# marqo-ai/marqo

Hardware: NVIDIA H100
Metric: embeddings/s (open_clip/ViT-L-14 image vectorise, batch 256 per GPU) (higher is better)
Workload: dtype bf16

## Files before the change

marqo_b200/csrc/gemm.cu:

```cuda
#include "gemm.cuh"

#include <mutex>

#include "ptx.cuh"

namespace mb {
namespace gemm {

constexpr int BM = 128;
constexpr int BN = 128;
constexpr int BK = 64;
constexpr int WG_K = 16;
constexpr int STAGES = 3;
constexpr int MMA_THREADS = 256;
constexpr uint32_t A_STAGE_BYTES = BM * BK * 2;
constexpr uint32_t B_STAGE_BYTES = BN * BK * 2;
constexpr uint32_t STAGE_BYTES = A_STAGE_BYTES + B_STAGE_BYTES;
constexpr uint32_t BARRIER_BYTES = 256;
constexpr size_t SMEM_BYTES = (size_t)STAGES * STAGE_BYTES + 1024  + BARRIER_BYTES + 2 * BN * 4 ;
constexpr int EPI_ROWS = BM / 2;
constexpr uint32_t EPI_BOX_BYTES = EPI_ROWS * 128;
static_assert(4 * EPI_BOX_BYTES == STAGE_BYTES, "a warpgroup's fp32 64 x 128 block is one ring stage");

template <bool GATHER>
constexpr int threads() { return MMA_THREADS + (GATHER ? 128 : 32); }

struct Params {
    int M, N, K;
    int tiles_n;
    Epilogue ep;
    const uint8_t* img;
    int g;
    int patch;
    int row_bytes;
    int seg;
    int kbpd;
    float nscale[3], nshift[3];
};

__device__ __forceinline__ float ex2_approx(float x) {
    float y;
    asm("ex2.approx.ftz.f32 %0, %1;" : "=f"(y) : "f"(x));
    return y;
}

__device__ __forceinline__ float gelu_erf(float x) {
    const float a = x * 0.70710678118654752440f;
    const float t = fabsf(a);
    const float s = a * a;
    float r = fmaf(-2.49374837e-5f, t, 5.52836593e-4f);
    const float u = fmaf(-5.60337594e-3f, t, 3.49920232e-2f);
    r = fmaf(r, s, u);
    r = fmaf(r, t, -1.54047912e-1f);
    r = fmaf(r, t, -9.15890168e-1f);
    r = fmaf(r, t, -1.85700115e-1f);
    r = fmaf(r, t, -1.44269504f * t);
    const float e = copysignf(1.0f - ex2_approx(r), a);
    const float hx = 0.5f * x;
    return fmaf(hx, e, hx);
}

__device__ __forceinline__ __half2 gelu_erf_h2(__half2 x) {
    const __half2 a = __hmul2(x, __float2half2_rn(0.70710678118654752440f));
    const __half2 t = __habs2(a);
    const __half2 s = __hmul2(a, a);
    __half2 r = __hfma2(__float2half2_rn(-2.49374837e-5f), t, __float2half2_rn(5.52836593e-4f));
    const __half2 u = __hfma2(__float2half2_rn(-5.60337594e-3f), t, __float2half2_rn(3.49920232e-2f));
    r = __hfma2(r, s, u);
    r = __hfma2(r, t, __float2half2_rn(-1.54047912e-1f));
    r = __hfma2(r, t, __float2half2_rn(-9.15890168e-1f));
    r = __hfma2(r, t, __float2half2_rn(-1.85700115e-1f));
    r = __hfma2(r, t, __hmul2(t, __float2half2_rn(-1.44269504f)));
    const __half2 e = h2exp2(r);
    const __half2 om = __hsub2(__float2half2_rn(1.0f), e);
    const uint32_t eb = (*reinterpret_cast<const uint32_t*>(&om) & 0x7fff7fffu) | (*reinterpret_cast<const uint32_t*>(&a) & 0x80008000u);
    const __half2 erfv = *reinterpret_cast<const __half2*>(&eb);
    const __half2 hx = __hmul2(x, __float2half2_rn(0.5f));
    return __hfma2(hx, erfv, hx);
}

__device__ __forceinline__ float quick_gelu(float x) {
    return x / (1.0f + ex2_approx(-1.702f * 1.44269504f * x));
}

__device__ __forceinline__ uint32_t pack_bf16x2(float lo, float hi) {
    __nv_bfloat162 v = __floats2bfloat162_rn(lo, hi);
    return *reinterpret_cast<uint32_t*>(&v);
}

__device__ __forceinline__ uint32_t sw128_offset(int row, int unit) {
    return (uint32_t)row * 128u + (uint32_t)((unit ^ (row & 7)) << 4);
}

template <int ELEM>
__device__ __forceinline__ uint32_t epi_offset(int row, int col) {
    constexpr int BOX_COLS = 128 / ELEM;
    const int byte = (col % BOX_COLS) * ELEM;
    return (uint32_t)(col / BOX_COLS) * EPI_BOX_BYTES + sw128_offset(row, byte >> 4) + (uint32_t)(byte & 15);
}

__device__ __forceinline__ void warpgroup_sync(int wg) {
    if (wg == 0)
        ptx::bar_sync<1, 128>();
    else
        ptx::bar_sync<2, 128>();
}

template <bool GATHER, bool STAGED>
__global__ void __launch_bounds__(threads<GATHER>(), GATHER ? 1 : 2)
gemm_kernel(const __grid_constant__ CUtensorMap tmap_a, const __grid_constant__ CUtensorMap tmap_b,
            const __grid_constant__ CUtensorMap tmap_r, const __grid_constant__ CUtensorMap tmap_o, Params p) {
    static_assert(!(GATHER && STAGED), "the patch embed scatters token rows: register epilogue");
    extern __shared__ uint8_t smem_raw[];
    uint8_t* smem = reinterpret_cast<uint8_t*>((reinterpret_cast<uintptr_t>(smem_raw) + 1023) & ~uintptr_t(1023));
    uint64_t* full = reinterpret_cast<uint64_t*>(smem + (size_t)STAGES * STAGE_BYTES);
    uint64_t* empty = full + STAGES;
    float* bias_s = reinterpret_cast<float*>(smem + (size_t)STAGES * STAGE_BYTES + BARRIER_BYTES);

    const int warp = __shfl_sync(0xffffffffu, threadIdx.x >> 5, 0);
    const int lane = threadIdx.x & 31;
    const int tile_m = blockIdx.x / p.tiles_n, tile_n = blockIdx.x % p.tiles_n;
    const int m0 = tile_m * BM, n0 = tile_n * BN;
    const int kblocks = p.K / BK;

    if (threadIdx.x == MMA_THREADS) {
        ptx::prefetch_tmap(&tmap_b);
        if (!GATHER) ptx::prefetch_tmap(&tmap_a);
        if (STAGED) {
            ptx::prefetch_tmap(&tmap_o);
            if (p.ep.residual) ptx::prefetch_tmap(&tmap_r);
        }
        for (int i = 0; i < STAGES; ++i) {
            ptx::mbar_init(&full[i], GATHER ? 1 + 128 : 1);
            ptx::mbar_init(&empty[i], MMA_THREADS / 32);
        }
        ptx::fence_barrier_init();
    }
    __syncthreads();

    if (threadIdx.x >= MMA_THREADS) {
        const int pt = threadIdx.x - MMA_THREADS;
        if (!GATHER && pt >= 32) return;
        const uint8_t* prow = nullptr;
        if (GATHER) {
            const int r = m0 + pt;
            if (r < p.M) {
                const int gg = p.g * p.g;
                const int b = r / gg, pi = r - b * gg;
                const int py = pi / p.g, px = pi - py * p.g;
                prow = p.img + ((size_t)b * p.g * p.patch + (size_t)py * p.patch) * p.row_bytes + (size_t)px * p.patch * 3;
            }
        }
        for (int kb = 0; kb < kblocks; ++kb) {
            const int stage = kb % STAGES;
            const uint32_t phase = (uint32_t)(kb / STAGES) & 1u;
            uint8_t* sa = smem + (size_t)stage * STAGE_BYTES;
            uint8_t* sb = sa + A_STAGE_BYTES;
            ptx::mbar_wait(&empty[stage], phase ^ 1);
            if (pt == 0) {
                ptx::mbar_arrive_expect_tx(&full[stage], GATHER ? B_STAGE_BYTES : STAGE_BYTES);
                if (!GATHER) ptx::tma_load_2d(sa, &tmap_a, &full[stage], kb * BK, m0, ptx::kEvictNormal);
                ptx::tma_load_2d(sb, &tmap_b, &full[stage], kb * BK, n0, ptx::kEvictLast);
            }
            if (GATHER) {
                const int dy = kb / p.kbpd, j0 = (kb - dy * p.kbpd) * 64;
                const uint8_t* src = prow ? prow + (size_t)dy * p.row_bytes + j0 : nullptr;
                int c = j0 % 3;
#pragma unroll 1
                for (int u = 0; u < 8; ++u) {
                    uint32_t w[4];
#pragma unroll
                    for (int e = 0; e < 4; ++e) {
                        float v[2];
#pragma unroll
                        for (int h = 0; h < 2; ++h) {
                            const int j = u * 8 + e * 2 + h;
                            v[h] = (src != nullptr && j0 + j < p.seg) ? fmaf((float)__ldg(src + j), p.nscale[c], p.nshift[c]) : 0.f;
                            c = c == 2 ? 0 : c + 1;
                        }
                        w[e] = pack_bf16x2(v[0], v[1]);
                    }
                    *reinterpret_cast<uint4*>(sa + sw128_offset(pt, u)) = make_uint4(w[0], w[1], w[2], w[3]);
                }
                ptx::fence_proxy_async_smem();
                ptx::mbar_arrive(&full[stage]);
            }
        }
        if (STAGED) {
            for (int wg = 0; wg < 2; ++wg) {
                const int kb = kblocks + wg;
                const int stage = kb % STAGES;
                uint8_t* s = smem + (size_t)stage * STAGE_BYTES;
                ptx::mbar_wait(&empty[stage], ((uint32_t)(kb / STAGES) & 1u) ^ 1);
                if (pt != 0) continue;
                const int row0 = m0 + EPI_ROWS * wg;
                const int boxes = p.ep.residual != nullptr && row0 < p.M ? min(4, (p.N - n0) / 32) : 0;
                ptx::mbar_arrive_expect_tx(&full[stage], (uint32_t)boxes * EPI_BOX_BYTES);
                for (int b = 0; b < boxes; ++b)
                    ptx::tma_load_2d(s + b * EPI_BOX_BYTES, &tmap_r, &full[stage], n0 + 32 * b, row0, ptx::kEvictNormal);
            }
        }
        return;
    }

    const int wg = warp >> 2;
    const Epilogue& ep = p.ep;
    float bias_t = 0.f;
    if (STAGED && ep.bias != nullptr && n0 + (int)(threadIdx.x & 127) < p.N) bias_t = __ldg(ep.bias + n0 + (threadIdx.x & 127));
    float acc[BN / 2];
#pragma unroll
    for (int i = 0; i < BN / 2; ++i) acc[i] = 0.f;
    for (int kb = 0; kb < kblocks; ++kb) {
        const int stage = kb % STAGES;
        ptx::mbar_wait(&full[stage], (uint32_t)(kb / STAGES) & 1u);
        const uint32_t a_base = ptx::smem_u32(smem + (size_t)stage * STAGE_BYTES) + wg * (64 * 128);
        const uint32_t b_base = ptx::smem_u32(smem + (size_t)stage * STAGE_BYTES + A_STAGE_BYTES);
        ptx::wgmma_fence();
#pragma unroll
        for (int k = 0; k < BK / WG_K; ++k)
            ptx::wgmma_m64n128k16_bf16(acc, ptx::make_desc_k_sw128(a_base + k * WG_K * 2),
                                       ptx::make_desc_k_sw128(b_base + k * WG_K * 2), (kb | k) != 0 ? 1u : 0u);
        ptx::wgmma_commit();
        ptx::wgmma_wait<1>();
        if (kb > 0 && lane == 0) ptx::mbar_arrive(&empty[(kb - 1) % STAGES]);
    }
    ptx::wgmma_wait<0>();

    if constexpr (STAGED) {
        const int t = threadIdx.x & 127;
        float* wbias = bias_s + wg * BN;
        wbias[t] = bias_t;
        const int kb = kblocks + wg;
        ptx::mbar_wait(&full[kb % STAGES], (uint32_t)(kb / STAGES) & 1u);
        uint8_t* tile = smem + (size_t)(kb % STAGES) * STAGE_BYTES;
        warpgroup_sync(wg);
        const int rbase = (warp & 3) * 16 + (lane >> 2);
        const bool half_gelu = ep.act == ACT_GELU && !ep.act_fp32 && !ep.out_fp32;
#pragma unroll
        for (int i = 0; i < BN / 8; ++i) {
            const int col = 8 * i + 2 * (lane & 3);
            const float2 bv = *reinterpret_cast<const float2*>(wbias + col);
#pragma unroll
            for (int h = 0; h < 2; ++h) {
                const int r = rbase + 8 * h;
                float x0 = acc[4 * i + 2 * h] + bv.x, x1 = acc[4 * i + 2 * h + 1] + bv.y;
                if (half_gelu) {
                    const float2 y = __half22float2(gelu_erf_h2(__floats2half2_rn(x0, x1)));
                    *reinterpret_cast<uint32_t*>(tile + epi_offset<2>(r, col)) = pack_bf16x2(y.x, y.y);
                    continue;
                }
                if (ep.act == ACT_GELU) {
                    x0 = gelu_erf(x0);
                    x1 = gelu_erf(x1);
                } else if (ep.act == ACT_QUICKGELU) {
                    x0 = quick_gelu(x0);
                    x1 = quick_gelu(x1);
                }
                if (ep.out_fp32) {
                    float2* dst = reinterpret_cast<float2*>(tile + epi_offset<4>(r, col));
                    if (ep.residual) {
                        const float2 rv = *dst;
                        x0 += rv.x;
                        x1 += rv.y;
                    }
                    *dst = make_float2(x0, x1);
                } else {
                    *reinterpret_cast<uint32_t*>(tile + epi_offset<2>(r, col)) = pack_bf16x2(x0, x1);
                }
            }
        }
        ptx::fence_proxy_async_smem();
        warpgroup_sync(wg);
        const int row0 = m0 + EPI_ROWS * wg;
        if (t == 0 && row0 < p.M) {
            const int box_cols = ep.out_fp32 ? 32 : 64;
            for (int b = 0; b * box_cols < BN && n0 + b * box_cols < p.N; ++b)
                ptx::tma_store_2d(&tmap_o, tile + b * EPI_BOX_BYTES, n0 + b * box_cols, row0);
            ptx::tma_store_commit();
            ptx::tma_store_wait_read<0>();
        }
    } else {
        const int rbase = m0 + wg * 64 + (warp & 3) * 16 + (lane >> 2);
        long long orow[2];
        bool rok[2];
#pragma unroll
        for (int h = 0; h < 2; ++h) {
            const int r = rbase + 8 * h;
            const int b = r / ep.remap_group;
            rok[h] = r < p.M;
            orow[h] = (long long)b * (ep.remap_group + 1) + 1 + (r - b * ep.remap_group);
        }
#pragma unroll
        for (int i = 0; i < BN / 8; ++i) {
            const int col = n0 + 8 * i + 2 * (lane & 3);
            if (col >= p.N) continue;
            float2 bv = make_float2(0.f, 0.f);
            if (ep.bias) bv = __ldg(reinterpret_cast<const float2*>(ep.bias + col));
#pragma unroll
            for (int h = 0; h < 2; ++h) {
                if (!rok[h]) continue;
                const int r = rbase + 8 * h;
                float x0 = acc[4 * i + 2 * h] + bv.x, x1 = acc[4 * i + 2 * h + 1] + bv.y;
                if (ep.act == ACT_GELU) {
                    x0 = gelu_erf(x0);
                    x1 = gelu_erf(x1);
                } else if (ep.act == ACT_QUICKGELU) {
                    x0 = quick_gelu(x0);
                    x1 = quick_gelu(x1);
                }
                if (ep.rowbias) {
                    const float2 pb =
                        __ldg(reinterpret_cast<const float2*>(ep.rowbias + (size_t)(1 + r % ep.remap_group) * p.N + col));
                    x0 += pb.x;
                    x1 += pb.y;
                }
                *reinterpret_cast<float2*>(static_cast<float*>(ep.out) + orow[h] * ep.ldo + col) = make_float2(x0, x1);
            }
        }
    }
}

void configure() {
    static std::once_flag once;
    std::call_once(once, [] {
        const auto attr = cudaFuncAttributeMaxDynamicSharedMemorySize;
        MB_CUDA(cudaFuncSetAttribute(gemm_kernel<false, true>, attr, (int)SMEM_BYTES));
        MB_CUDA(cudaFuncSetAttribute(gemm_kernel<false, false>, attr, (int)SMEM_BYTES));
        MB_CUDA(cudaFuncSetAttribute(gemm_kernel<true, false>, attr, (int)SMEM_BYTES));
    });
}

template <bool GATHER, bool STAGED>
static void launch_tiles(const __nv_bfloat16* A, int lda, const __nv_bfloat16* W, int M, int N, int K, const Epilogue& ep,
                         cudaStream_t stream, const PatchGather* pg = nullptr) {
    Params p{};
    if (GATHER) {
        p.img = pg->img;
        p.patch = pg->patch;
        p.g = pg->S / pg->patch;
        p.row_bytes = 3 * pg->S;
        p.seg = 3 * pg->patch;
        p.kbpd = patch_gather_kbpd(pg->patch);
        for (int c = 0; c < 3; ++c) {
            p.nscale[c] = (float)(1.0 / (255.0 * (double)pg->std[c]));
            p.nshift[c] = (float)(-(double)pg->mean[c] / (double)pg->std[c]);
        }
    }
    p.M = M;
    p.N = N;
    p.K = K;
    p.tiles_n = (N + BN - 1) / BN;
    p.ep = ep;
    const long long tiles = (long long)((M + BM - 1) / BM) * p.tiles_n;
    if (tiles > 0x7fffffffLL) fail(B200_ERR_UNSUPPORTED, "gemm: %lld tiles is too many", tiles);
    CUtensorMap tb = make_tmap_2d(W, CU_TENSOR_MAP_DATA_TYPE_BFLOAT16, 2, (uint64_t)K, (uint64_t)N, (uint64_t)K * 2, BK, BN,
                                  CU_TENSOR_MAP_SWIZZLE_128B);
    CUtensorMap ta = GATHER ? tb
                            : make_tmap_2d(A, CU_TENSOR_MAP_DATA_TYPE_BFLOAT16, 2, (uint64_t)K, (uint64_t)M,
                                           (uint64_t)lda * 2, BK, BM, CU_TENSOR_MAP_SWIZZLE_128B);
    CUtensorMap tr = tb, to = tb;
    if (STAGED) {
        if (ep.residual)
            tr = make_tmap_2d(ep.residual, CU_TENSOR_MAP_DATA_TYPE_FLOAT32, 4, (uint64_t)N, (uint64_t)M,
                              (uint64_t)ep.ldr * 4, 32, EPI_ROWS, CU_TENSOR_MAP_SWIZZLE_128B);
        to = ep.out_fp32 ? make_tmap_2d(ep.out, CU_TENSOR_MAP_DATA_TYPE_FLOAT32, 4, (uint64_t)N, (uint64_t)M,
                                        (uint64_t)ep.ldo * 4, 32, EPI_ROWS, CU_TENSOR_MAP_SWIZZLE_128B)
                         : make_tmap_2d(ep.out, CU_TENSOR_MAP_DATA_TYPE_BFLOAT16, 2, (uint64_t)N, (uint64_t)M,
                                        (uint64_t)ep.ldo * 2, 64, EPI_ROWS, CU_TENSOR_MAP_SWIZZLE_128B);
    }
    gemm_kernel<GATHER, STAGED><<<(unsigned)tiles, threads<GATHER>(), SMEM_BYTES, stream>>>(ta, tb, tr, to, p);
    MB_CUDA(cudaGetLastError());
}

bool patch_gather_supported(int S, int patch) {
    return S > 0 && patch > 0 && S % patch == 0;
}

void launch_patch_embed(const PatchGather& pg, const __nv_bfloat16* Wg, int N, const Epilogue& ep, int sms,
                        cudaStream_t stream) {
    (void)sms;
    if (pg.n <= 0 || N <= 0) return;
    if (!patch_gather_supported(pg.S, pg.patch))
        fail(B200_ERR_INTERNAL, "patch gather: image %d / patch %d is not supported", pg.S, pg.patch);
    if (N % 32 != 0 || ep.ldo % 8 != 0) fail(B200_ERR_INTERNAL, "patch gather: N = %d, ldo = %d", N, ep.ldo);
    if (ep.remap_group <= 0 || ep.residual != nullptr || !ep.out_fp32)
        fail(B200_ERR_INTERNAL, "patch gather: token scatter to fp32 output without residual only");
    configure();
    const int g = pg.S / pg.patch;
    const long long M = (long long)pg.n * g * g;
    if (M > 0x7fffffffLL) fail(B200_ERR_INVALID_ARG, "patch gather: batch of %d images is too large", pg.n);
    launch_tiles<true, false>(nullptr, 0, Wg, (int)M, N, patch_gather_k(pg.patch), ep, stream, &pg);
}

void launch(const __nv_bfloat16* A, int lda, const __nv_bfloat16* W, int M, int N, int K, const Epilogue& ep, int sms,
            cudaStream_t stream) {
    (void)sms;
    if (M <= 0 || N <= 0) return;
    if (K <= 0 || K % BK != 0) fail(B200_ERR_INTERNAL, "gemm: K = %d must be a positive multiple of %d", K, BK);
    if (N % 32 != 0) fail(B200_ERR_INTERNAL, "gemm: N = %d must be a multiple of 32", N);
    if (lda % 8 != 0 || ep.ldo % 8 != 0) fail(B200_ERR_INTERNAL, "gemm: leading dimensions must be multiples of 8");
    if (ep.remap_group > 0) {
        if (ep.residual != nullptr || !ep.out_fp32)
            fail(B200_ERR_INTERNAL, "gemm: token scatter to fp32 output without residual only");
        configure();
        launch_tiles<false, false>(A, lda, W, M, N, K, ep, stream);
        return;
    }
    if ((reinterpret_cast<uintptr_t>(ep.out) & 15) != 0) fail(B200_ERR_INTERNAL, "gemm: output not 16-byte aligned");
    if (ep.rowbias != nullptr) fail(B200_ERR_INTERNAL, "gemm: the positional bias goes with the token scatter");
    if (ep.residual != nullptr &&
        (!ep.out_fp32 || ep.ldr % 4 != 0 || (reinterpret_cast<uintptr_t>(ep.residual) & 15) != 0))
        fail(B200_ERR_INTERNAL, "gemm: the residual needs an fp32 output, ldr %% 4 == 0 and 16-byte alignment");
    configure();
    launch_tiles<false, true>(A, lda, W, M, N, K, ep, stream);
}

}
}
```

marqo_b200/csrc/ptx.cuh:

```cuda
#pragma once
#include <cstdint>
#include <cstdio>
#include <cuda.h>
#include <cuda_runtime.h>

namespace ptx {

__device__ __forceinline__ uint32_t smem_u32(const void* p) {
    return static_cast<uint32_t>(__cvta_generic_to_shared(p));
}

__device__ __forceinline__ uint32_t lane_id() {
    uint32_t l;
    asm volatile("mov.u32 %0, %%laneid;" : "=r"(l));
    return l;
}

__device__ __forceinline__ uint64_t globaltimer_ns() {
    uint64_t t;
    asm volatile("mov.u64 %0, %%globaltimer;" : "=l"(t));
    return t;
}

__device__ __forceinline__ bool elect_one() {
    uint32_t pred;
    asm volatile(
        "{\n"
        ".reg .pred p;\n"
        "elect.sync _|p, 0xffffffff;\n"
        "selp.u32 %0, 1, 0, p;\n"
        "}\n"
        : "=r"(pred));
    return pred != 0;
}

__device__ __forceinline__ void mbar_init(uint64_t* bar, uint32_t count) {
    asm volatile("mbarrier.init.shared::cta.b64 [%0], %1;" ::"r"(smem_u32(bar)), "r"(count) : "memory");
}
__device__ __forceinline__ void fence_barrier_init() {
    asm volatile("fence.mbarrier_init.release.cluster;" ::: "memory");
}
__device__ __forceinline__ void fence_proxy_async_smem() {
    asm volatile("fence.proxy.async.shared::cta;" ::: "memory");
}
__device__ __forceinline__ void mbar_arrive_expect_tx(uint64_t* bar, uint32_t bytes) {
    asm volatile("mbarrier.arrive.expect_tx.shared::cta.b64 _, [%0], %1;" ::"r"(smem_u32(bar)), "r"(bytes)
                 : "memory");
}
__device__ __forceinline__ void mbar_arrive(uint64_t* bar) {
    asm volatile("mbarrier.arrive.shared::cta.b64 _, [%0];" ::"r"(smem_u32(bar)) : "memory");
}
__device__ __forceinline__ bool mbar_try_wait(uint64_t* bar, uint32_t parity) {
    uint32_t ok;
    asm volatile(
        "{\n"
        ".reg .pred p;\n"
        "mbarrier.try_wait.parity.shared::cta.b64 p, [%1], %2;\n"
        "selp.u32 %0, 1, 0, p;\n"
        "}\n"
        : "=r"(ok)
        : "r"(smem_u32(bar)), "r"(parity)
        : "memory");
    return ok != 0;
}
__device__ __forceinline__ void mbar_wait(uint64_t* bar, uint32_t parity) {
    if (mbar_try_wait(bar, parity)) return;
    uint64_t t0 = globaltimer_ns();
    uint32_t spins = 0;
    while (!mbar_try_wait(bar, parity)) {
        if ((++spins & 0x3ff) == 0 && globaltimer_ns() - t0 > 4000000000ull) __trap();
    }
}

constexpr uint64_t kEvictNormal = 0x1000000000000000ull;
constexpr uint64_t kEvictFirst = 0x12F0000000000000ull;
constexpr uint64_t kEvictLast = 0x14F0000000000000ull;

__device__ __forceinline__ void prefetch_tmap(const CUtensorMap* tmap) {
    asm volatile("prefetch.tensormap [%0];" ::"l"(reinterpret_cast<uint64_t>(tmap)) : "memory");
}

__device__ __forceinline__ void tma_load_2d(void* smem_dst, const CUtensorMap* tmap, uint64_t* bar, int32_t c0,
                                            int32_t c1, uint64_t cache_hint) {
    asm volatile(
        "cp.async.bulk.tensor.2d.shared::cluster.global.tile.mbarrier::complete_tx::bytes.L2::cache_hint"
        " [%0], [%1, {%3, %4}], [%2], %5;"
        ::"r"(smem_u32(smem_dst)), "l"(reinterpret_cast<uint64_t>(tmap)), "r"(smem_u32(bar)), "r"(c0), "r"(c1),
        "l"(cache_hint)
        : "memory");
}

__device__ __forceinline__ void tma_store_2d(const CUtensorMap* tmap, const void* smem_src, int32_t c0, int32_t c1) {
    asm volatile("cp.async.bulk.tensor.2d.global.shared::cta.tile.bulk_group [%0, {%2, %3}], [%1];" ::"l"(
                     reinterpret_cast<uint64_t>(tmap)),
                 "r"(smem_u32(smem_src)), "r"(c0), "r"(c1)
                 : "memory");
}
__device__ __forceinline__ void tma_store_commit() { asm volatile("cp.async.bulk.commit_group;" ::: "memory"); }
template <int N>
__device__ __forceinline__ void tma_store_wait_read() {
    asm volatile("cp.async.bulk.wait_group.read %0;" ::"n"(N) : "memory");
}
template <int N>
__device__ __forceinline__ void tma_store_wait() {
    asm volatile("cp.async.bulk.wait_group %0;" ::"n"(N) : "memory");
}

__device__ __forceinline__ uint64_t make_desc_k_sw128(uint32_t smem_addr) {
    uint64_t d = 0;
    d |= static_cast<uint64_t>((smem_addr & 0x3FFFF) >> 4);
    d |= static_cast<uint64_t>(1) << 16;
    d |= static_cast<uint64_t>(1024 >> 4) << 32;
    d |= static_cast<uint64_t>(1) << 62;
    return d;
}

__device__ __forceinline__ uint64_t make_desc_mn_sw128(uint32_t smem_addr, uint32_t lbo_bytes) {
    uint64_t d = 0;
    d |= static_cast<uint64_t>((smem_addr & 0x3FFFF) >> 4);
    d |= static_cast<uint64_t>((lbo_bytes >> 4) & 0x3FFF) << 16;
    d |= static_cast<uint64_t>(1024 >> 4) << 32;
    d |= static_cast<uint64_t>(1) << 62;
    return d;
}

__device__ __forceinline__ uint64_t make_desc_k_sw64(uint32_t smem_addr) {
    uint64_t d = 0;
    d |= static_cast<uint64_t>((smem_addr & 0x3FFFF) >> 4);
    d |= static_cast<uint64_t>(1) << 16;
    d |= static_cast<uint64_t>(512 >> 4) << 32;
    d |= static_cast<uint64_t>(2) << 62;
    return d;
}

__device__ __forceinline__ uint64_t make_desc_mn_sw64(uint32_t smem_addr, uint32_t lbo_bytes) {
    uint64_t d = 0;
    d |= static_cast<uint64_t>((smem_addr & 0x3FFFF) >> 4);
    d |= static_cast<uint64_t>((lbo_bytes >> 4) & 0x3FFF) << 16;
    d |= static_cast<uint64_t>(512 >> 4) << 32;
    d |= static_cast<uint64_t>(2) << 62;
    return d;
}

__device__ __forceinline__ void wgmma_fence() { asm volatile("wgmma.fence.sync.aligned;" ::: "memory"); }
__device__ __forceinline__ void wgmma_commit() { asm volatile("wgmma.commit_group.sync.aligned;" ::: "memory"); }
template <int N>
__device__ __forceinline__ void wgmma_wait() {
    asm volatile("wgmma.wait_group.sync.aligned %0;" ::"n"(N) : "memory");
}

__device__ __forceinline__ void wgmma_m64n128k16_f16(float (&d)[64], uint64_t desc_a, uint64_t desc_b, uint32_t scale_d) {
    asm volatile(
        "{\n"
        ".reg .pred p;\n"
        "setp.ne.b32 p, %66, 0;\n"
        "wgmma.mma_async.sync.aligned.m64n128k16.f32.f16.f16 "
        "{"
        "%0, %1, %2, %3, %4, %5, %6, %7, %8, %9, %10, %11, %12, %13, %14, %15, "
        "%16, %17, %18, %19, %20, %21, %22, %23, %24, %25, %26, %27, %28, %29, %30, %31, "
        "%32, %33, %34, %35, %36, %37, %38, %39, %40, %41, %42, %43, %44, %45, %46, %47, "
        "%48, %49, %50, %51, %52, %53, %54, %55, %56, %57, %58, %59, %60, %61, %62, %63"
        "}, %64, %65, p, 1, 1, 0, 0;\n"
        "}\n"
        : "+f"(d[0]), "+f"(d[1]), "+f"(d[2]), "+f"(d[3]), "+f"(d[4]), "+f"(d[5]), "+f"(d[6]), "+f"(d[7]),
          "+f"(d[8]), "+f"(d[9]), "+f"(d[10]), "+f"(d[11]), "+f"(d[12]), "+f"(d[13]), "+f"(d[14]), "+f"(d[15]),
          "+f"(d[16]), "+f"(d[17]), "+f"(d[18]), "+f"(d[19]), "+f"(d[20]), "+f"(d[21]), "+f"(d[22]), "+f"(d[23]),
          "+f"(d[24]), "+f"(d[25]), "+f"(d[26]), "+f"(d[27]), "+f"(d[28]), "+f"(d[29]), "+f"(d[30]), "+f"(d[31]),
          "+f"(d[32]), "+f"(d[33]), "+f"(d[34]), "+f"(d[35]), "+f"(d[36]), "+f"(d[37]), "+f"(d[38]), "+f"(d[39]),
          "+f"(d[40]), "+f"(d[41]), "+f"(d[42]), "+f"(d[43]), "+f"(d[44]), "+f"(d[45]), "+f"(d[46]), "+f"(d[47]),
          "+f"(d[48]), "+f"(d[49]), "+f"(d[50]), "+f"(d[51]), "+f"(d[52]), "+f"(d[53]), "+f"(d[54]), "+f"(d[55]),
          "+f"(d[56]), "+f"(d[57]), "+f"(d[58]), "+f"(d[59]), "+f"(d[60]), "+f"(d[61]), "+f"(d[62]), "+f"(d[63])
        : "l"(desc_a), "l"(desc_b), "r"(scale_d));
}
__device__ __forceinline__ void wgmma_m64n128k16_bf16(float (&d)[64], uint64_t desc_a, uint64_t desc_b, uint32_t scale_d) {
    asm volatile(
        "{\n"
        ".reg .pred p;\n"
        "setp.ne.b32 p, %66, 0;\n"
        "wgmma.mma_async.sync.aligned.m64n128k16.f32.bf16.bf16 "
        "{"
        "%0, %1, %2, %3, %4, %5, %6, %7, %8, %9, %10, %11, %12, %13, %14, %15, "
        "%16, %17, %18, %19, %20, %21, %22, %23, %24, %25, %26, %27, %28, %29, %30, %31, "
        "%32, %33, %34, %35, %36, %37, %38, %39, %40, %41, %42, %43, %44, %45, %46, %47, "
        "%48, %49, %50, %51, %52, %53, %54, %55, %56, %57, %58, %59, %60, %61, %62, %63"
        "}, %64, %65, p, 1, 1, 0, 0;\n"
        "}\n"
        : "+f"(d[0]), "+f"(d[1]), "+f"(d[2]), "+f"(d[3]), "+f"(d[4]), "+f"(d[5]), "+f"(d[6]), "+f"(d[7]),
          "+f"(d[8]), "+f"(d[9]), "+f"(d[10]), "+f"(d[11]), "+f"(d[12]), "+f"(d[13]), "+f"(d[14]), "+f"(d[15]),
          "+f"(d[16]), "+f"(d[17]), "+f"(d[18]), "+f"(d[19]), "+f"(d[20]), "+f"(d[21]), "+f"(d[22]), "+f"(d[23]),
          "+f"(d[24]), "+f"(d[25]), "+f"(d[26]), "+f"(d[27]), "+f"(d[28]), "+f"(d[29]), "+f"(d[30]), "+f"(d[31]),
          "+f"(d[32]), "+f"(d[33]), "+f"(d[34]), "+f"(d[35]), "+f"(d[36]), "+f"(d[37]), "+f"(d[38]), "+f"(d[39]),
          "+f"(d[40]), "+f"(d[41]), "+f"(d[42]), "+f"(d[43]), "+f"(d[44]), "+f"(d[45]), "+f"(d[46]), "+f"(d[47]),
          "+f"(d[48]), "+f"(d[49]), "+f"(d[50]), "+f"(d[51]), "+f"(d[52]), "+f"(d[53]), "+f"(d[54]), "+f"(d[55]),
          "+f"(d[56]), "+f"(d[57]), "+f"(d[58]), "+f"(d[59]), "+f"(d[60]), "+f"(d[61]), "+f"(d[62]), "+f"(d[63])
        : "l"(desc_a), "l"(desc_b), "r"(scale_d));
}
__device__ __forceinline__ void wgmma_m64n64k16_bf16_rs_tb(float (&d)[32], const uint32_t (&a)[4], uint64_t desc_b, uint32_t scale_d) {
    asm volatile(
        "{\n"
        ".reg .pred p;\n"
        "setp.ne.b32 p, %37, 0;\n"
        "wgmma.mma_async.sync.aligned.m64n64k16.f32.bf16.bf16 "
        "{"
        "%0, %1, %2, %3, %4, %5, %6, %7, %8, %9, %10, %11, %12, %13, %14, %15, "
        "%16, %17, %18, %19, %20, %21, %22, %23, %24, %25, %26, %27, %28, %29, %30, %31"
        "}, {%32, %33, %34, %35}, %36, p, 1, 1, 1;\n"
        "}\n"
        : "+f"(d[0]), "+f"(d[1]), "+f"(d[2]), "+f"(d[3]), "+f"(d[4]), "+f"(d[5]), "+f"(d[6]), "+f"(d[7]),
          "+f"(d[8]), "+f"(d[9]), "+f"(d[10]), "+f"(d[11]), "+f"(d[12]), "+f"(d[13]), "+f"(d[14]), "+f"(d[15]),
          "+f"(d[16]), "+f"(d[17]), "+f"(d[18]), "+f"(d[19]), "+f"(d[20]), "+f"(d[21]), "+f"(d[22]), "+f"(d[23]),
          "+f"(d[24]), "+f"(d[25]), "+f"(d[26]), "+f"(d[27]), "+f"(d[28]), "+f"(d[29]), "+f"(d[30]), "+f"(d[31])
        : "r"(a[0]), "r"(a[1]), "r"(a[2]), "r"(a[3]), "l"(desc_b), "r"(scale_d));
}
__device__ __forceinline__ void wgmma_m64n32k16_bf16_rs_tb(float (&d)[16], const uint32_t (&a)[4], uint64_t desc_b, uint32_t scale_d) {
    asm volatile(
        "{\n"
        ".reg .pred p;\n"
        "setp.ne.b32 p, %21, 0;\n"
        "wgmma.mma_async.sync.aligned.m64n32k16.f32.bf16.bf16 "
        "{"
        "%0, %1, %2, %3, %4, %5, %6, %7, %8, %9, %10, %11, %12, %13, %14, %15"
        "}, {%16, %17, %18, %19}, %20, p, 1, 1, 1;\n"
        "}\n"
        : "+f"(d[0]), "+f"(d[1]), "+f"(d[2]), "+f"(d[3]), "+f"(d[4]), "+f"(d[5]), "+f"(d[6]), "+f"(d[7]),
          "+f"(d[8]), "+f"(d[9]), "+f"(d[10]), "+f"(d[11]), "+f"(d[12]), "+f"(d[13]), "+f"(d[14]), "+f"(d[15])
        : "r"(a[0]), "r"(a[1]), "r"(a[2]), "r"(a[3]), "l"(desc_b), "r"(scale_d));
}
template <int ID, int COUNT>
__device__ __forceinline__ void bar_sync() {
    asm volatile("bar.sync %0, %1;" ::"n"(ID), "n"(COUNT) : "memory");
}

}
```

Baseline: 1877.

## Add persistent warp-specialized 128x256 GEMM kernel for large-K projections

Adds a persistent GEMM kernel with a 128x256 tile using m64n256k16 wgmma, a single-thread TMA producer warpgroup with reduced registers via setmaxnreg, and two consumer warpgroups with double epilogue buffers. It also adds residual TMA loads, L2 prefetch of the residual and a packed fp16 GELU path for bf16 outputs. It is dispatched when K >= 1024, N is a multiple of 256 and there are at least as many tiles as SMs. The aim is higher operand reuse per tile and less launch and tail overhead for the big ViT-L MLP and attention projections. The cost is heavy register pressure (128 fp32 accumulators per thread) and a serialized epilogue that is not overlapped with the next tile's MMA.

```diff
diff --git a/marqo_b200/csrc/gemm.cu b/marqo_b200/csrc/gemm.cu
--- a/marqo_b200/csrc/gemm.cu
+++ b/marqo_b200/csrc/gemm.cu
@@ -22,12 +22,23 @@
 constexpr uint32_t EPI_BOX_BYTES = EPI_ROWS * 128;
 static_assert(4 * EPI_BOX_BYTES == STAGE_BYTES, "a warpgroup's fp32 64 x 128 block is one ring stage");
 
+constexpr int P_BN = 256;
+constexpr int P_STAGES = 3;
+constexpr uint32_t P_STAGE_BYTES = A_STAGE_BYTES + P_BN * BK * 2;
+constexpr uint32_t P_RING_BYTES = P_STAGES * P_STAGE_BYTES;
+constexpr uint32_t EPI_BYTES = 4 * EPI_BOX_BYTES;
+constexpr int PERSISTENT_THREADS = 128 + MMA_THREADS;
+constexpr int ACT_GELU_H2 = 3;
+constexpr size_t P_SMEM_BYTES = 1024  + P_RING_BYTES + 2 * EPI_BYTES + 2 * P_BN * 4 + BARRIER_BYTES;
+static_assert(P_SMEM_BYTES <= 227 * 1024, "over the opt-in shared memory of an H100 CTA");
+static_assert(P_BN * 2 * EPI_ROWS == EPI_BYTES, "a warpgroup's bf16 64 x 256 block is one epilogue buffer");
+
 template <bool GATHER>
 constexpr int threads() { return MMA_THREADS + (GATHER ? 128 : 32); }
 
 struct Params {
     int M, N, K;
-    int tiles_n;
+    int tiles_m, tiles_n;
     Epilogue ep;
     const uint8_t* img;
     int g;
@@ -320,6 +331,201 @@
     }
 }
 
+template <bool OUT_FP32, int ACT>
+__global__ void __launch_bounds__(PERSISTENT_THREADS, 1)
+gemm_persistent_kernel(const __grid_constant__ CUtensorMap tmap_a, const __grid_constant__ CUtensorMap tmap_b,
+                       const __grid_constant__ CUtensorMap tmap_r, const __grid_constant__ CUtensorMap tmap_o, Params p) {
+    extern __shared__ uint8_t smem_raw[];
+    uint8_t* smem = reinterpret_cast<uint8_t*>((reinterpret_cast<uintptr_t>(smem_raw) + 1023) & ~uintptr_t(1023));
+    uint8_t* epi_s = smem + P_RING_BYTES;
+    float* bias_s = reinterpret_cast<float*>(epi_s + 2 * EPI_BYTES);
+    uint64_t* full = reinterpret_cast<uint64_t*>(bias_s + 2 * P_BN);
+    uint64_t* empty = full + P_STAGES;
+    uint64_t* epi_full = empty + P_STAGES;
+
+    const int tiles = p.tiles_m * p.tiles_n;
+    const int kblocks = p.K / BK;
+    const Epilogue& ep = p.ep;
+    const bool has_res = ep.residual != nullptr;
+
+    if (threadIdx.x == 0) {
+        ptx::prefetch_tmap(&tmap_a);
+        ptx::prefetch_tmap(&tmap_b);
+        ptx::prefetch_tmap(&tmap_o);
+        if (has_res) ptx::prefetch_tmap(&tmap_r);
+        for (int i = 0; i < P_STAGES; ++i) {
+            ptx::mbar_init(&full[i], 1);
+            ptx::mbar_init(&empty[i], MMA_THREADS / 32);
+        }
+        ptx::mbar_init(&epi_full[0], 1);
+        ptx::mbar_init(&epi_full[1], 1);
+        ptx::fence_barrier_init();
+    }
+    __syncthreads();
+
+    if (threadIdx.x < 128) {
+        ptx::setmaxnreg_dec<40>();
+        if (threadIdx.x != 0) return;
+        uint32_t it = 0;
+        for (int tile = blockIdx.x; tile < tiles; tile += gridDim.x) {
+            const int m0 = (tile / p.tiles_n) * BM, n0 = (tile % p.tiles_n) * P_BN;
+            for (int kb = 0; kb < kblocks; ++kb, ++it) {
+                const int stage = it % P_STAGES;
+                uint8_t* sa = smem + (size_t)stage * P_STAGE_BYTES;
+                ptx::mbar_wait(&empty[stage], ((it / P_STAGES) & 1u) ^ 1);
+                ptx::mbar_arrive_expect_tx(&full[stage], P_STAGE_BYTES);
+                ptx::tma_load_2d(sa, &tmap_a, &full[stage], kb * BK, m0, ptx::kEvictNormal);
+                ptx::tma_load_2d(sa + A_STAGE_BYTES, &tmap_b, &full[stage], kb * BK, n0, ptx::kEvictLast);
+            }
+        }
+        return;
+    }
+
+    ptx::setmaxnreg_inc<232>();
+    const int wg = (threadIdx.x >> 7) - 1;
+    const int t = threadIdx.x & 127;
+    const int warp = t >> 5, lane = t & 31;
+    uint8_t* buf = epi_s + wg * EPI_BYTES;
+    float* wbias = bias_s + wg * P_BN;
+    const uint32_t buf_s = ptx::smem_u32(buf), wbias_s = ptx::smem_u32(wbias);
+    const int rbase = warp * 16 + (lane >> 2);
+    static_assert(!(OUT_FP32 && ACT == ACT_GELU_H2), "packed fp16 GELU is for bf16 outputs");
+    constexpr int HALVES = P_BN / 128;
+    uint32_t it = 0, epi_phase = 0;
+
+    auto load_residual = [&](int row0, int c0) {
+        const int boxes = row0 < p.M && c0 < p.N ? min(4, (p.N - c0) / 32) : 0;
+        ptx::mbar_arrive_expect_tx(&epi_full[wg], (uint32_t)boxes * EPI_BOX_BYTES);
+        for (int b = 0; b < boxes; ++b)
+            ptx::tma_load_2d(buf + b * EPI_BOX_BYTES, &tmap_r, &epi_full[wg], c0 + 32 * b, row0, ptx::kEvictNormal);
+    };
+
+    for (int tile = blockIdx.x; tile < tiles; tile += gridDim.x) {
+        const int m0 = (tile / p.tiles_n) * BM, n0 = (tile % p.tiles_n) * P_BN;
+        const int row0 = m0 + EPI_ROWS * wg;
+        float bias_r[P_BN / 128];
+#pragma unroll
+        for (int j = 0; j < P_BN / 128; ++j) {
+            const int c = n0 + t + 128 * j;
+            bias_r[j] = ep.bias != nullptr && c < p.N ? __ldg(ep.bias + c) : 0.f;
+        }
+        float acc[P_BN / 2];
+#pragma unroll
+        for (int i = 0; i < P_BN / 2; ++i) acc[i] = 0.f;
+        for (int kb = 0; kb < kblocks; ++kb, ++it) {
+            const int stage = it % P_STAGES;
+            ptx::mbar_wait(&full[stage], (it / P_STAGES) & 1u);
+            const uint32_t a_base = ptx::smem_u32(smem + (size_t)stage * P_STAGE_BYTES) + wg * (64 * 128);
+            const uint32_t b_base = ptx::smem_u32(smem + (size_t)stage * P_STAGE_BYTES + A_STAGE_BYTES);
+            ptx::wgmma_fence();
+#pragma unroll
+            for (int k = 0; k < BK / WG_K; ++k) {
+                const uint64_t da = ptx::make_desc_k_sw128(a_base + k * WG_K * 2);
+                const uint64_t db = ptx::make_desc_k_sw128(b_base + k * WG_K * 2);
+                ptx::wgmma_m64n256k16_bf16(acc, da, db, (kb | k) != 0 ? 1u : 0u);
+            }
+            ptx::wgmma_commit();
+            ptx::wgmma_wait<1>();
+            if (kb > 0 && lane == 0) ptx::mbar_arrive(&empty[(it - 1) % P_STAGES]);
+            if (kb == 0 && t == 0) {
+                ptx::tma_store_wait_read<0>();
+                if (has_res) {
+                    load_residual(row0, n0);
+                    if (row0 < p.M)
+                        for (int b = 0; b < 4 && n0 + 128 + 32 * b < p.N; ++b)
+                            ptx::tma_prefetch_l2_2d(&tmap_r, n0 + 128 + 32 * b, row0);
+                }
+            }
+        }
+        ptx::wgmma_wait<0>();
+        if (lane == 0) ptx::mbar_arrive(&empty[(it - 1) % P_STAGES]);
+
+#pragma unroll
+        for (int j = 0; j < P_BN / 128; ++j) wbias[t + 128 * j] = bias_r[j];
+        warpgroup_sync(wg);
+        if constexpr (!OUT_FP32) {
+#pragma unroll
+            for (int i = 0; i < P_BN / 8; ++i) {
+                const int col = 8 * i + 2 * (lane & 3);
+                const float2 bv = ptx::ld_shared_f32x2(wbias_s + 4 * col);
+#pragma unroll
+                for (int h = 0; h < 2; ++h) {
+                    const int r = rbase + 8 * h;
+                    float x0 = acc[4 * i + 2 * h] + bv.x, x1 = acc[4 * i + 2 * h + 1] + bv.y;
+                    if constexpr (ACT == ACT_GELU_H2) {
+                        const float2 y = __half22float2(gelu_erf_h2(__floats2half2_rn(x0, x1)));
+                        x0 = y.x;
+                        x1 = y.y;
+                    } else if constexpr (ACT == ACT_GELU) {
+                        x0 = gelu_erf(x0);
+                        x1 = gelu_erf(x1);
+                    } else if constexpr (ACT == ACT_QUICKGELU) {
+                        x0 = quick_gelu(x0);
+                        x1 = quick_gelu(x1);
+                    }
+                    ptx::st_shared_u32(buf_s + epi_offset<2>(r, col), pack_bf16x2(x0, x1));
+                }
+            }
+            ptx::fence_proxy_async_smem();
+            warpgroup_sync(wg);
+            if (t == 0 && row0 < p.M) {
+                for (int b = 0; b < P_BN / 64 && n0 + 64 * b < p.N; ++b)
+                    ptx::tma_store_2d(&tmap_o, buf + b * EPI_BOX_BYTES, n0 + 64 * b, row0);
+                ptx::tma_store_commit();
+            }
+        } else {
+#pragma unroll
+            for (int hf = 0; hf < HALVES; ++hf) {
+                if (hf > 0) {
+                    if (t == 0) {
+                        ptx::tma_store_wait_read<0>();
+                        if (has_res) load_residual(row0, n0 + 128 * hf);
+                    }
+                    if (!has_res) warpgroup_sync(wg);
+                }
+                if (has_res) {
+                    ptx::mbar_wait(&epi_full[wg], epi_phase);
+                    epi_phase ^= 1;
+                }
+#pragma unroll
+                for (int i = 0; i < 16; ++i) {
+                    const int col = 8 * i + 2 * (lane & 3);
+                    const int ai = 4 * (16 * hf + i);
+                    const float2 bv = ptx::ld_shared_f32x2(wbias_s + 4 * (128 * hf + col));
+#pragma unroll
+                    for (int h = 0; h < 2; ++h) {
+                        const int r = rbase + 8 * h;
+                        float x0 = acc[ai + 2 * h] + bv.x, x1 = acc[ai + 2 * h + 1] + bv.y;
+                        if constexpr (ACT == ACT_GELU) {
+                            x0 = gelu_erf(x0);
+                            x1 = gelu_erf(x1);
+                        } else if constexpr (ACT == ACT_QUICKGELU) {
+                            x0 = quick_gelu(x0);
+                            x1 = quick_gelu(x1);
+                        }
+                        const uint32_t dst = buf_s + epi_offset<4>(r, col);
+                        if (has_res) {
+                            const float2 rv = ptx::ld_shared_f32x2(dst);
+                            x0 += rv.x;
+                            x1 += rv.y;
+                        }
+                        ptx::st_shared_f32x2(dst, x0, x1);
+                    }
+                }
+                ptx::fence_proxy_async_smem();
+                warpgroup_sync(wg);
+                const int c0 = n0 + 128 * hf;
+                if (t == 0 && row0 < p.M && c0 < p.N) {
+                    for (int b = 0; b < 4 && c0 + 32 * b < p.N; ++b)
+                        ptx::tma_store_2d(&tmap_o, buf + b * EPI_BOX_BYTES, c0 + 32 * b, row0);
+                    ptx::tma_store_commit();
+                }
+            }
+        }
+    }
+    if (t == 0) ptx::tma_store_wait_read<0>();
+}
+
 void configure() {
     static std::once_flag once;
     std::call_once(once, [] {
@@ -327,6 +533,13 @@
         MB_CUDA(cudaFuncSetAttribute(gemm_kernel<false, true>, attr, (int)SMEM_BYTES));
         MB_CUDA(cudaFuncSetAttribute(gemm_kernel<false, false>, attr, (int)SMEM_BYTES));
         MB_CUDA(cudaFuncSetAttribute(gemm_kernel<true, false>, attr, (int)SMEM_BYTES));
+        MB_CUDA(cudaFuncSetAttribute(gemm_persistent_kernel<false, ACT_NONE>, attr, (int)P_SMEM_BYTES));
+        MB_CUDA(cudaFuncSetAttribute(gemm_persistent_kernel<false, ACT_GELU>, attr, (int)P_SMEM_BYTES));
+        MB_CUDA(cudaFuncSetAttribute(gemm_persistent_kernel<false, ACT_QUICKGELU>, attr, (int)P_SMEM_BYTES));
+        MB_CUDA(cudaFuncSetAttribute(gemm_persistent_kernel<false, ACT_GELU_H2>, attr, (int)P_SMEM_BYTES));
+        MB_CUDA(cudaFuncSetAttribute(gemm_persistent_kernel<true, ACT_NONE>, attr, (int)P_SMEM_BYTES));
+        MB_CUDA(cudaFuncSetAttribute(gemm_persistent_kernel<true, ACT_GELU>, attr, (int)P_SMEM_BYTES));
+        MB_CUDA(cudaFuncSetAttribute(gemm_persistent_kernel<true, ACT_QUICKGELU>, attr, (int)P_SMEM_BYTES));
     });
 }
 
@@ -372,6 +585,56 @@
     MB_CUDA(cudaGetLastError());
 }
 
+template <bool OUT_FP32, int ACT>
+static void launch_persistent(const __nv_bfloat16* A, int lda, const __nv_bfloat16* W, int M, int N, int K,
+                              const Epilogue& ep, int sms, cudaStream_t stream) {
+    Params p{};
+    p.M = M;
+    p.N = N;
+    p.K = K;
+    p.tiles_m = (M + BM - 1) / BM;
+    p.tiles_n = (N + P_BN - 1) / P_BN;
+    p.ep = ep;
+    const long long tiles = (long long)p.tiles_m * p.tiles_n;
+    if (tiles > 0x7fffffffLL) fail(B200_ERR_UNSUPPORTED, "gemm: %lld tiles is too many", tiles);
+    CUtensorMap ta = make_tmap_2d(A, CU_TENSOR_MAP_DATA_TYPE_BFLOAT16, 2, (uint64_t)K, (uint64_t)M, (uint64_t)lda * 2,
+                                  BK, BM, CU_TENSOR_MAP_SWIZZLE_128B);
+    CUtensorMap tb = make_tmap_2d(W, CU_TENSOR_MAP_DATA_TYPE_BFLOAT16, 2, (uint64_t)K, (uint64_t)N, (uint64_t)K * 2, BK,
+                                  P_BN, CU_TENSOR_MAP_SWIZZLE_128B);
+    CUtensorMap tr = ep.residual ? make_tmap_2d(ep.residual, CU_TENSOR_MAP_DATA_TYPE_FLOAT32, 4, (uint64_t)N, (uint64_t)M,
+                                                (uint64_t)ep.ldr * 4, 32, EPI_ROWS, CU_TENSOR_MAP_SWIZZLE_128B)
+                                 : tb;
+    CUtensorMap to = ep.out_fp32 ? make_tmap_2d(ep.out, CU_TENSOR_MAP_DATA_TYPE_FLOAT32, 4, (uint64_t)N, (uint64_t)M,
+                                                (uint64_t)ep.ldo * 4, 32, EPI_ROWS, CU_TENSOR_MAP_SWIZZLE_128B)
+                                 : make_tmap_2d(ep.out, CU_TENSOR_MAP_DATA_TYPE_BFLOAT16, 2, (uint64_t)N, (uint64_t)M,
+                                                (uint64_t)ep.ldo * 2, 64, EPI_ROWS, CU_TENSOR_MAP_SWIZZLE_128B);
+    const int grid = (int)std::min<long long>(tiles, std::max(sms, 1));
+    gemm_persistent_kernel<OUT_FP32, ACT><<<grid, PERSISTENT_THREADS, P_SMEM_BYTES, stream>>>(ta, tb, tr, to, p);
+    MB_CUDA(cudaGetLastError());
+}
+
+static void launch_persistent(const __nv_bfloat16* A, int lda, const __nv_bfloat16* W, int M, int N, int K,
+                              const Epilogue& ep, int sms, cudaStream_t stream) {
+    const int act = ep.act == ACT_GELU && !ep.act_fp32 && !ep.out_fp32 ? ACT_GELU_H2 : ep.act;
+    if (ep.out_fp32) {
+        if (act == ACT_GELU)
+            launch_persistent<true, ACT_GELU>(A, lda, W, M, N, K, ep, sms, stream);
+        else if (act == ACT_QUICKGELU)
+            launch_persistent<true, ACT_QUICKGELU>(A, lda, W, M, N, K, ep, sms, stream);
+        else
+            launch_persistent<true, ACT_NONE>(A, lda, W, M, N, K, ep, sms, stream);
+    } else {
+        if (act == ACT_GELU_H2)
+            launch_persistent<false, ACT_GELU_H2>(A, lda, W, M, N, K, ep, sms, stream);
+        else if (act == ACT_GELU)
+            launch_persistent<false, ACT_GELU>(A, lda, W, M, N, K, ep, sms, stream);
+        else if (act == ACT_QUICKGELU)
+            launch_persistent<false, ACT_QUICKGELU>(A, lda, W, M, N, K, ep, sms, stream);
+        else
+            launch_persistent<false, ACT_NONE>(A, lda, W, M, N, K, ep, sms, stream);
+    }
+}
+
 bool patch_gather_supported(int S, int patch) {
     return S > 0 && patch > 0 && S % patch == 0;
 }
@@ -394,7 +657,6 @@
 
 void launch(const __nv_bfloat16* A, int lda, const __nv_bfloat16* W, int M, int N, int K, const Epilogue& ep, int sms,
             cudaStream_t stream) {
-    (void)sms;
     if (M <= 0 || N <= 0) return;
     if (K <= 0 || K % BK != 0) fail(B200_ERR_INTERNAL, "gemm: K = %d must be a positive multiple of %d", K, BK);
     if (N % 32 != 0) fail(B200_ERR_INTERNAL, "gemm: N = %d must be a multiple of 32", N);
@@ -412,8 +674,12 @@
         (!ep.out_fp32 || ep.ldr % 4 != 0 || (reinterpret_cast<uintptr_t>(ep.residual) & 15) != 0))
         fail(B200_ERR_INTERNAL, "gemm: the residual needs an fp32 output, ldr %% 4 == 0 and 16-byte alignment");
     configure();
-    launch_tiles<false, true>(A, lda, W, M, N, K, ep, stream);
-}
-
-}
-}
+    const long long tiles256 = (long long)((M + BM - 1) / BM) * (N / P_BN);
+    if (K >= 1024 && N % P_BN == 0 && tiles256 >= sms)
+        launch_persistent(A, lda, W, M, N, K, ep, sms, stream);
+    else
+        launch_tiles<false, true>(A, lda, W, M, N, K, ep, stream);
+}
+
+}
+}
diff --git a/marqo_b200/csrc/ptx.cuh b/marqo_b200/csrc/ptx.cuh
--- a/marqo_b200/csrc/ptx.cuh
+++ b/marqo_b200/csrc/ptx.cuh
@@ -8,6 +8,18 @@
 
 __device__ __forceinline__ uint32_t smem_u32(const void* p) {
     return static_cast<uint32_t>(__cvta_generic_to_shared(p));
+}
+
+__device__ __forceinline__ void st_shared_u32(uint32_t addr, uint32_t v) {
+    asm volatile("st.shared.b32 [%0], %1;" ::"r"(addr), "r"(v) : "memory");
+}
+__device__ __forceinline__ void st_shared_f32x2(uint32_t addr, float x, float y) {
+    asm volatile("st.shared.v2.f32 [%0], {%1, %2};" ::"r"(addr), "f"(x), "f"(y) : "memory");
+}
+__device__ __forceinline__ float2 ld_shared_f32x2(uint32_t addr) {
+    float2 v;
+    asm volatile("ld.shared.v2.f32 {%0, %1}, [%2];" : "=f"(v.x), "=f"(v.y) : "r"(addr) : "memory");
+    return v;
 }
 
 __device__ __forceinline__ uint32_t lane_id() {
@@ -90,6 +102,12 @@
         : "memory");
 }
 
+__device__ __forceinline__ void tma_prefetch_l2_2d(const CUtensorMap* tmap, int32_t c0, int32_t c1) {
+    asm volatile("cp.async.bulk.prefetch.tensor.2d.L2.global.tile [%0, {%1, %2}];" ::"l"(reinterpret_cast<uint64_t>(tmap)),
+                 "r"(c0), "r"(c1)
+                 : "memory");
+}
+
 __device__ __forceinline__ void tma_store_2d(const CUtensorMap* tmap, const void* smem_src, int32_t c0, int32_t c1) {
     asm volatile("cp.async.bulk.tensor.2d.global.shared::cta.tile.bulk_group [%0, {%2, %3}], [%1];" ::"l"(
                      reinterpret_cast<uint64_t>(tmap)),
@@ -195,6 +213,41 @@
           "+f"(d[56]), "+f"(d[57]), "+f"(d[58]), "+f"(d[59]), "+f"(d[60]), "+f"(d[61]), "+f"(d[62]), "+f"(d[63])
         : "l"(desc_a), "l"(desc_b), "r"(scale_d));
 }
+__device__ __forceinline__ void wgmma_m64n256k16_bf16(float (&d)[128], uint64_t desc_a, uint64_t desc_b, uint32_t scale_d) {
+    asm volatile(
+        "{\n"
+        ".reg .pred p;\n"
+        "setp.ne.b32 p, %130, 0;\n"
+        "wgmma.mma_async.sync.aligned.m64n256k16.f32.bf16.bf16 "
+        "{"
+        "%0, %1, %2, %3, %4, %5, %6, %7, %8, %9, %10, %11, %12, %13, %14, %15, "
+        "%16, %17, %18, %19, %20, %21, %22, %23, %24, %25, %26, %27, %28, %29, %30, %31, "
+        "%32, %33, %34, %35, %36, %37, %38, %39, %40, %41, %42, %43, %44, %45, %46, %47, "
+        "%48, %49, %50, %51, %52, %53, %54, %55, %56, %57, %58, %59, %60, %61, %62, %63, "
+        "%64, %65, %66, %67, %68, %69, %70, %71, %72, %73, %74, %75, %76, %77, %78, %79, "
+        "%80, %81, %82, %83, %84, %85, %86, %87, %88, %89, %90, %91, %92, %93, %94, %95, "
+        "%96, %97, %98, %99, %100, %101, %102, %103, %104, %105, %106, %107, %108, %109, %110, %111, "
+        "%112, %113, %114, %115, %116, %117, %118, %119, %120, %121, %122, %123, %124, %125, %126, %127"
+        "}, %128, %129, p, 1, 1, 0, 0;\n"
+        "}\n"
+        : "+f"(d[0]), "+f"(d[1]), "+f"(d[2]), "+f"(d[3]), "+f"(d[4]), "+f"(d[5]), "+f"(d[6]), "+f"(d[7]),
+          "+f"(d[8]), "+f"(d[9]), "+f"(d[10]), "+f"(d[11]), "+f"(d[12]), "+f"(d[13]), "+f"(d[14]), "+f"(d[15]),
+          "+f"(d[16]), "+f"(d[17]), "+f"(d[18]), "+f"(d[19]), "+f"(d[20]), "+f"(d[21]), "+f"(d[22]), "+f"(d[23]),
+          "+f"(d[24]), "+f"(d[25]), "+f"(d[26]), "+f"(d[27]), "+f"(d[28]), "+f"(d[29]), "+f"(d[30]), "+f"(d[31]),
+          "+f"(d[32]), "+f"(d[33]), "+f"(d[34]), "+f"(d[35]), "+f"(d[36]), "+f"(d[37]), "+f"(d[38]), "+f"(d[39]),
+          "+f"(d[40]), "+f"(d[41]), "+f"(d[42]), "+f"(d[43]), "+f"(d[44]), "+f"(d[45]), "+f"(d[46]), "+f"(d[47]),
+          "+f"(d[48]), "+f"(d[49]), "+f"(d[50]), "+f"(d[51]), "+f"(d[52]), "+f"(d[53]), "+f"(d[54]), "+f"(d[55]),
+          "+f"(d[56]), "+f"(d[57]), "+f"(d[58]), "+f"(d[59]), "+f"(d[60]), "+f"(d[61]), "+f"(d[62]), "+f"(d[63]),
+          "+f"(d[64]), "+f"(d[65]), "+f"(d[66]), "+f"(d[67]), "+f"(d[68]), "+f"(d[69]), "+f"(d[70]), "+f"(d[71]),
+          "+f"(d[72]), "+f"(d[73]), "+f"(d[74]), "+f"(d[75]), "+f"(d[76]), "+f"(d[77]), "+f"(d[78]), "+f"(d[79]),
+          "+f"(d[80]), "+f"(d[81]), "+f"(d[82]), "+f"(d[83]), "+f"(d[84]), "+f"(d[85]), "+f"(d[86]), "+f"(d[87]),
+          "+f"(d[88]), "+f"(d[89]), "+f"(d[90]), "+f"(d[91]), "+f"(d[92]), "+f"(d[93]), "+f"(d[94]), "+f"(d[95]),
+          "+f"(d[96]), "+f"(d[97]), "+f"(d[98]), "+f"(d[99]), "+f"(d[100]), "+f"(d[101]), "+f"(d[102]), "+f"(d[103]),
+          "+f"(d[104]), "+f"(d[105]), "+f"(d[106]), "+f"(d[107]), "+f"(d[108]), "+f"(d[109]), "+f"(d[110]), "+f"(d[111]),
+          "+f"(d[112]), "+f"(d[113]), "+f"(d[114]), "+f"(d[115]), "+f"(d[116]), "+f"(d[117]), "+f"(d[118]), "+f"(d[119]),
+          "+f"(d[120]), "+f"(d[121]), "+f"(d[122]), "+f"(d[123]), "+f"(d[124]), "+f"(d[125]), "+f"(d[126]), "+f"(d[127])
+        : "l"(desc_a), "l"(desc_b), "r"(scale_d));
+}
 __device__ __forceinline__ void wgmma_m64n64k16_bf16_rs_tb(float (&d)[32], const uint32_t (&a)[4], uint64_t desc_b, uint32_t scale_d) {
     asm volatile(
         "{\n"
@@ -226,6 +279,15 @@
           "+f"(d[8]), "+f"(d[9]), "+f"(d[10]), "+f"(d[11]), "+f"(d[12]), "+f"(d[13]), "+f"(d[14]), "+f"(d[15])
         : "r"(a[0]), "r"(a[1]), "r"(a[2]), "r"(a[3]), "l"(desc_b), "r"(scale_d));
 }
+template <int REGS>
+__device__ __forceinline__ void setmaxnreg_inc() {
+    asm volatile("setmaxnreg.inc.sync.aligned.u32 %0;" ::"n"(REGS));
+}
+template <int REGS>
+__device__ __forceinline__ void setmaxnreg_dec() {
+    asm volatile("setmaxnreg.dec.sync.aligned.u32 %0;" ::"n"(REGS));
+}
+
 template <int ID, int COUNT>
 __device__ __forceinline__ void bar_sync() {
     asm volatile("bar.sync %0, %1;" ::"n"(ID), "n"(COUNT) : "memory");
```

After: 2077 (median of 6 runs). 10.7% higher.
